# tayloraswift/swift-png

Measured on NVIDIA H100. Metric: MPixels/s decode (inflate+unfilter), higher is better.
Workload: dtype u8

## Files before the change

swift-png_b200/csrc/common.cuh:

```cuda
#pragma once

#ifdef PNGB200_EMU
#include "simt.h"
#else
#include <cuda_runtime.h>
#define PNGB200_DYN_SMEM(name) extern __shared__ __align__(16) unsigned char name[]
#endif
#include <stdint.h>

#include "../../include/pngb200.h"

namespace pngb200 {

struct StreamJob {
    const uint8_t* src;
    uint64_t       src_len;
    uint8_t*       dst;
    uint64_t       dst_cap;
    uint64_t       start_bit;
    uint64_t       start_out;
    int32_t        format;
    int32_t        phase;
    uint64_t       stop_bit;
    uint32_t       symbolic;
    uint32_t       may_switch;
    uint8_t*       scratch;
    uint64_t       scratch_cap;
};

struct StreamResult {
    int32_t  status;
    uint32_t err_a, err_b;
    uint32_t checksum;
    uint32_t blocks;
    uint32_t declared;
    uint64_t produced;
    uint64_t consumed_bits;
    uint64_t resume_bit;
    uint64_t resume_out;
    uint32_t trailer_seen;
    uint32_t phase;
    uint32_t stat_waves, stat_sync_rounds, stat_resolve_rounds, stat_fallback;
    uint64_t stat_tokens, stat_matches, stat_deferred;
    uint32_t ck_done;
    uint32_t pad_;
    uint64_t stat_cycles[12];
};

struct SwitchRecord {
    uint64_t out;
    uint64_t bytes;
};

struct ImageJob {
    const uint8_t*      filtered;
    uint8_t*            pixels;
    const StreamResult* inflated;
    uint64_t            filtered_len;
    uint32_t            width, height;
    uint32_t            pitch;
    uint8_t             volume, depth, interlaced, bpp;
};

__device__ __forceinline__ uint64_t usable_bytes(const StreamResult* r, uint64_t fallback)
{
    if (r == nullptr) return fallback;
    return r->status < 0 ? 0 : r->produced;
}

__device__ __forceinline__ unsigned lane_id() { return threadIdx.x & 31u; }

__device__ __forceinline__ uint32_t ld_volatile_u32(const uint32_t* p)
{
#ifdef PNGB200_EMU
    return *(const volatile uint32_t*)p;
#else
    uint32_t v;
    asm volatile("ld.volatile.global.u32 %0, [%1];" : "=r"(v) : "l"(p) : "memory");
    return v;
#endif
}
__device__ __forceinline__ void st_volatile_u32(uint32_t* p, uint32_t v)
{
#ifdef PNGB200_EMU
    *(volatile uint32_t*)p = v;
#else
    asm volatile("st.volatile.global.u32 [%0], %1;" ::"l"(p), "r"(v) : "memory");
#endif
}

}
```

swift-png_b200/csrc/huffman.cuh:

```cuda
#pragma once

#include "common.cuh"

namespace pngb200 {

enum : uint32_t { K_LIT = 0, K_BASE = 1, K_EOB = 2, K_PTR = 3, K_INVALID = 4 };
enum : uint32_t { E_COPY = 1u << 9, E_SPECIAL = 1u << 10, E_PTR = 1u << 11, E_INVALID = 2u << 11 };
__device__ __forceinline__ uint32_t mk_entry(uint32_t kind, uint32_t len, uint32_t extra, uint32_t value)
{
    uint32_t e = len | (len + extra) << 4 | value << 16;
    if (kind == K_BASE) e |= E_COPY;
    else if (kind == K_EOB) e |= E_SPECIAL;
    else if (kind == K_PTR) e |= E_SPECIAL | E_PTR;
    else if (kind == K_INVALID) e |= E_SPECIAL | E_INVALID;
    return e;
}
__device__ __forceinline__ uint32_t e_len(uint32_t e) { return e & 15u; }
__device__ __forceinline__ uint32_t e_skip(uint32_t e) { return (e >> 4) & 31u; }
__device__ __forceinline__ uint32_t e_extra(uint32_t e) { return e_skip(e) - e_len(e); }
__device__ __forceinline__ uint32_t e_kind(uint32_t e)
{
    return (e & E_SPECIAL) ? (((e >> 11) & 3u) == 0 ? K_EOB : ((e >> 11) & 3u) == 1 ? K_PTR : K_INVALID)
                           : ((e >> 9) & 1u);
}
__device__ __forceinline__ uint32_t e_value(uint32_t e) { return e >> 16; }

constexpr int LIT_ROOT  = 10;
constexpr int DIST_ROOT = 8;
constexpr int META_ROOT = 7;
constexpr int LIT_CAP   = (1 << LIT_ROOT) + 512;
constexpr int DIST_CAP  = (1 << DIST_ROOT) + 512;
constexpr int META_CAP  = 1 << META_ROOT;

__constant__ uint16_t c_len_base[29]  = {3, 4, 5, 6, 7, 8, 9, 10, 11, 13, 15, 17, 19, 23, 27,
                                         31, 35, 43, 51, 59, 67, 83, 99, 115, 131, 163, 195, 227, 258};
__constant__ uint8_t  c_len_extra[29] = {0, 0, 0, 0, 0, 0, 0, 0, 1, 1, 1, 1, 2, 2, 2,
                                         2, 3, 3, 3, 3, 4, 4, 4, 4, 5, 5, 5, 5, 0};
__constant__ uint16_t c_dist_base[30] = {1, 2, 3, 4, 5, 7, 9, 13, 17, 25, 33, 49, 65, 97, 129, 193,
                                         257, 385, 513, 769, 1025, 1537, 2049, 3073, 4097, 6145,
                                         8193, 12289, 16385, 24577};
__constant__ uint8_t  c_dist_extra[30] = {0, 0, 0, 0, 1, 1, 2, 2, 3, 3, 4, 4, 5, 5, 6, 6,
                                          7, 7, 8, 8, 9, 9, 10, 10, 11, 11, 12, 12, 13, 13};
__constant__ uint8_t  c_clen_order[19] = {16, 17, 18, 0, 8, 7, 9, 6, 10, 5, 11, 4, 12, 3, 13, 2, 14, 1, 15};

enum : int { ALPHA_LITLEN = 0, ALPHA_DIST = 1, ALPHA_META = 2 };

struct HuffScratch {
    uint32_t count[16];
    uint32_t first[16];
    uint32_t offs[16];
    uint32_t running[16];
    uint16_t sorted[320];
    uint32_t sub_alloc;
    int32_t  status;
    int32_t  stub;
};

__device__ __forceinline__ uint32_t symbol_entry(int alphabet, uint32_t sym, uint32_t len)
{
    if (alphabet == ALPHA_LITLEN) {
        if (sym < 256) return mk_entry(K_LIT, len, 0, sym);
        if (sym == 256) return mk_entry(K_EOB, len, 0, 0);
        if (sym < 286) return mk_entry(K_BASE, len, c_len_extra[sym - 257], c_len_base[sym - 257]);
        return mk_entry(K_INVALID, len, 0, sym);
    } else if (alphabet == ALPHA_DIST) {
        if (sym < 30) return mk_entry(K_BASE, len, c_dist_extra[sym], c_dist_base[sym]);
        return mk_entry(K_INVALID, len, 0, sym);
    }
    return mk_entry(K_LIT, len, 0, sym);
}

template <int ROOT, int CAP>
__device__ void build_table(uint32_t* table, const uint8_t* lens, int nsym, int alphabet,
                            HuffScratch* S, int tid, int nt)
{
    auto sync = [&]() {
        if (nt == 32) __syncwarp();
        else __syncthreads();
    };
    if (tid < 16) { S->count[tid] = 0; S->running[tid] = 0; }
    if (tid == 0) { S->sub_alloc = 1u << ROOT; S->status = 0; S->stub = -2; }
    sync();
    for (int s = tid; s < nsym; s += nt) atomicAdd(&S->count[lens[s]], 1u);
    sync();
    if (tid == 0) {
        int nonzero = nsym - (int)S->count[0];
        bool stub = false;
        if (alphabet == ALPHA_DIST) {
            if (nonzero == 0) { S->stub = -1; stub = true; }
            else if (nonzero == 1 && S->count[1] == 1) { S->stub = 0; stub = true; }
        }
        long interior = 1;
        uint32_t code = 0, off = 0;
        S->count[0] = 0;
        for (int l = 1; l <= 15; ++l) {
            code = (code + S->count[l - 1]) << 1;
            S->first[l] = code;
            S->offs[l] = off;
            off += S->count[l];
            interior = 2 * interior - (long)S->count[l];
        }
        if (!stub && interior != 0)
            S->status = alphabet == ALPHA_META ? PNGB200_ERR_CODELENGTH_HUFFMAN_TABLE
                                               : PNGB200_ERR_HUFFMAN_TABLE;
    }
    sync();
    if (S->status != 0) return;
    if (tid < 32) {
        for (int base = 0; base < nsym; base += 32) {
            int      s = base + tid;
            uint32_t l = s < nsym ? lens[s] : 0;
            unsigned peers = __match_any_sync(0xffffffffu, l);
            if (l) {
                uint32_t rank = __popc(peers & ((1u << tid) - 1u));
                uint32_t r0   = S->running[l];
                S->sorted[S->offs[l] + r0 + rank] = (uint16_t)s;
                __syncwarp(peers);
                if (rank == 0) S->running[l] = r0 + __popc(peers);
            }
            __syncwarp();
        }
    }
    sync();
    for (int i = tid; i < (1 << ROOT); i += nt) {
        uint32_t v = __brev((uint32_t)i) >> (32 - ROOT);
        uint32_t e = 0;
        bool     found = false;
#pragma unroll
        for (int l = 1; l <= ROOT; ++l) {
            uint32_t d = (v >> (ROOT - l)) - S->first[l];
            if (!found && d < S->count[l]) {
                e = symbol_entry(alphabet, S->sorted[S->offs[l] + d], (uint32_t)l);
                found = true;
            }
        }
        if (!found) {
            int maxl = 0;
            for (int l = ROOT + 1; l <= 15; ++l) {
                uint32_t lo = v << (l - ROOT), hi = (v + 1) << (l - ROOT);
                uint32_t a = S->first[l], b = a + S->count[l];
                if (S->count[l] && lo < b && a < hi) maxl = l;
            }
            if (maxl == 0) {
                e = mk_entry(K_INVALID, 0, 0, 0);
            } else {
                int      k    = maxl - ROOT;
                uint32_t slot = atomicAdd(&S->sub_alloc, 1u << k);
                if (slot + (1u << k) > (uint32_t)CAP) {
                    S->status = PNGB200_ERR_INTERNAL;
                    e = mk_entry(K_INVALID, 0, 0, 0);
                } else {
                    e = mk_entry(K_PTR, ROOT, (uint32_t)k, slot);
                    const uint32_t inv = mk_entry(K_INVALID, 0, 0, 0);
                    for (uint32_t j = 0; j < (1u << k); ++j) table[slot + j] = inv;
                }
            }
        }
        table[i] = e;
    }
    sync();
// ... 30 lines not shown
```

swift-png_b200/csrc/inflate_cells.cuh:

```cuda
#pragma once

#include "inflate_stream.cuh"

namespace pngb200 {

constexpr int      CL_CTAS_PER_SM = 3;
constexpr uint32_t CL_SLOTS       = 16000;
constexpr uint32_t CL_CAP         = CL_SLOTS - 16;
constexpr uint32_t CL_INWAVE      = 0xc000u;
constexpr uint32_t CL_WINDOW_BIAS = 0x8100u;
constexpr uint32_t CL_MIN_SUBS    = 32;
constexpr uint32_t CL_TCAP        = 64;
constexpr uint32_t CL_WCAP        = 64;
constexpr uint64_t CL_SCRATCH     = (uint64_t)WV_THREADS * (CL_TCAP + CL_WCAP) * sizeof(uint32_t);

struct ClShared {
    SerialShared ser;
    uint32_t     words[WV_SMEM_WORDS];
    uint32_t     mask[8 * WV_THREADS];
    uint32_t     pf_tail[16];
    uint32_t     exit_[WV_THREADS];
    uint32_t     wpos_[WV_THREADS];
    uint32_t     wn_[WV_THREADS];
    uint64_t     cross_[WV_THREADS];
// ... 17 lines not shown
static_assert(sizeof(ClShared) <= (228 * 1024 - CL_CTAS_PER_SM * 1024) / CL_CTAS_PER_SM, "CTAs per SM");
static_assert(CL_SLOTS <= 16384 && CL_SLOTS % 16 == 0, "14-bit cell index");

#ifdef PNGB200_EMU
inline void     sts16(saddr_t a, uint32_t v) { *(volatile uint16_t*)a = (uint16_t)v; }
inline uint32_t lds16(saddr_t a) { return *(volatile uint16_t*)a; }
inline void     sts32(saddr_t a, uint32_t v) { *(volatile uint32_t*)a = v; }
inline void     reds_or(saddr_t a, uint32_t v) { *(volatile uint32_t*)a |= v; }
#else
__device__ __forceinline__ void sts16(uint32_t a, uint32_t v)
{
    asm volatile("st.shared.u16 [%0], %1;" ::"r"(a), "h"((uint16_t)v) : "memory");
}
__device__ __forceinline__ uint32_t lds16(uint32_t a)
{
    uint16_t v;
    asm volatile("ld.shared.u16 %0, [%1];" : "=h"(v) : "r"(a) : "memory");
    return v;
}
__device__ __forceinline__ void sts32(uint32_t a, uint32_t v)
{
    asm volatile("st.shared.u32 [%0], %1;" ::"r"(a), "r"(v) : "memory");
}
__device__ __forceinline__ void reds_or(uint32_t a, uint32_t v)
{
    asm volatile("red.shared.or.b32 [%0], %1;" ::"r"(a), "r"(v) : "memory");
}
#endif
typedef saddr_t cellp_t;

__device__ __forceinline__ uint32_t cl_decode(FastBits& b, saddr_t lit, saddr_t dst, uint32_t& tok, uint32_t& nbytes, uint32_t& cp)
{
    const uint32_t bits = b.peek();
    uint32_t e = lds32(lit + ((bits & ((1u << LIT_ROOT) - 1u)) << 2));
    if (e & E_SPECIAL) {
        if ((e & (E_PTR | E_INVALID)) == E_PTR) e = lds32(lit + (((e >> 16) + bfe32(bits, LIT_ROOT, e_skip(e) - LIT_ROOT)) << 2));
        if (e & E_SPECIAL) {
            if (e & E_INVALID) return PF_BAD;
            b.skip(e_len(e));
            return PF_EOB;
        }
    }
    const uint32_t len = e & 15u, skipn = (e >> 4) & 31u;
    const uint32_t run = (e >> 16) + bfe32(bits, len, skipn - len);
    b.skip(skipn);
    cp = (e >> 9) & 1u;
    const uint32_t dbits = b.peek();
    uint32_t d = lds32(dst + ((dbits & ((1u << DIST_ROOT) - 1u)) << 2));
    if (d & E_SPECIAL) {
        if ((d & (E_PTR | E_INVALID)) == E_PTR) d = lds32(dst + (((d >> 16) + bfe32(dbits, DIST_ROOT, e_skip(d) - DIST_ROOT)) << 2));
        if (cp && (d & E_SPECIAL)) return PF_BAD;
    }
    const uint32_t dlen = d & 15u, dskip = (d >> 4) & 31u;
    const uint32_t dist = (d >> 16) + bfe32(dbits, dlen, dskip - dlen);
    b.skip(cp ? dskip : 0u);
    tok = run << 16 | (cp ? dist : 0u);
    nbytes = cp ? run : 1u;
    return 0;
}
__device__ __forceinline__ uint32_t tok_bytes(uint32_t v) { return (v & 0xffffu) ? v >> 16 : 1u; }

__device__ __forceinline__ void cells_copy(cellp_t ch, uint32_t j, uint32_t run, uint32_t dist, uint32_t jbeg)
{
    const int32_t src = (int32_t)j - (int32_t)dist;
    const saddr_t to = ch + 2 * j;
    if (src >= (int32_t)jbeg || src + (int32_t)run <= (int32_t)jbeg) {
        const uint32_t code = src >= (int32_t)jbeg ? CL_INWAVE + (uint32_t)src
                                                   : (uint32_t)((int32_t)CL_WINDOW_BIAS + src - (int32_t)jbeg);
        sts16(to, code);
        sts16(to + 2, code + 1);
        sts16(to + 4, code + 2);
        if (run > 3) sts16(to + 6, code + 3);
        for (uint32_t k = 4; k < run; ++k) sts16(to + 2 * k, code + k);
        return;
    }
    const uint32_t nwin = (uint32_t)((int32_t)jbeg - src);
    uint32_t code = (uint32_t)((int32_t)CL_WINDOW_BIAS + src - (int32_t)jbeg);
    uint32_t k = 0;
    for (; k < nwin; ++k) sts16(to + 2 * k, code + k);
    code = CL_INWAVE + (uint32_t)src;
    for (; k < run; ++k) sts16(to + 2 * k, code + k);
}

constexpr uint32_t CL_HDR_POS = 4480;

template <class Shared>
__device__ int cl_header_preamble(Shared& sh, uint64_t hbase_bit, uint64_t pos, uint64_t total_bits, int lane, WvHeader& out,
                                  uint32_t& rel_out)
{
    const uint32_t* const W = sh.words;
    auto get = [&](uint32_t rel, uint32_t n) -> uint32_t {
        const uint32_t w = rel >> 5;
        const uint32_t v = __funnelshift_r(W[w], W[w + 1], rel & 31u);
        return n >= 32 ? v : v & ((1u << n) - 1u);
    };
    uint32_t rel = (uint32_t)(pos - hbase_bit);
    if (pos + 3 > total_bits) return 0;
    const uint32_t h3 = get(rel, 3);
    rel += 3;
    out.status = PNGB200_OK;
    out.final = (int32_t)(h3 & 1u);
    out.type = (int32_t)(h3 >> 1);
    out.stored = 0;
    out.nlit = out.ndist = 0;
    if (out.type == 3) return 0;
    if (out.type == 0) {
        const uint64_t boundary = (pos + 3 + 7) & ~(uint64_t)7;
        if (boundary + 32 > total_bits) return 0;
        const uint32_t v = get((uint32_t)(boundary - hbase_bit), 32);
        const uint32_t l = v & 0xffffu, m = v >> 16;
        if (l != (~m & 0xffffu)) return 0;
        out.stored = l;
        out.pos = boundary + 32;
        return 1;
    }
    uint8_t* const lens = sh.ser.lens;
    if (out.type == 1) {
        for (int k = lane; k < 320; k += 32) lens[k] = k < 144 ? 8 : k < 256 ? 9 : k < 280 ? 7 : k < 288 ? 8 : 5;
        out.nlit = 288;
        out.ndist = 32;
        out.pos = pos + 3;
        __syncwarp();
        return 1;
    }
    if (pos + 17 > total_bits) return 0;
    const uint32_t v = get(rel, 14);
    rel += 14;
    const int nlit = 257 + (int)(v & 31u), ndist = 1 + (int)((v >> 5) & 31u), nclen = 4 + (int)(v >> 10);
    if (nlit > 286) return 0;
    if (lane < 19) lens[lane] = 0;
    __syncwarp();
    if (lane < nclen) lens[c_clen_order[lane]] = (uint8_t)get(rel + 3u * (uint32_t)lane, 3);
    rel += 3u * (uint32_t)nclen;
    __syncwarp();
    build_table<META_ROOT, META_CAP>(sh.ser.meta, lens, 19, ALPHA_META, &sh.ser.scratch, lane, 32);
    if (sh.ser.scratch.status) return 0;
    __syncwarp();
    if (rel + CL_HDR_POS + 64 > 32u * WV_HDR_WORDS) return 0;
    out.nlit = nlit;
    out.ndist = ndist;
    rel_out = rel;
    return 2;
}

__global__ void __launch_bounds__(WV_THREADS, CL_CTAS_PER_SM) inflate_cells_kernel(WvParams P)
{
    PNGB200_DYN_SMEM(cl_smem);
    ClShared& sh = *reinterpret_cast<ClShared*>(cl_smem);
    const uint32_t t    = threadIdx.x;
    const unsigned lane = lane_id(), warp = t >> 5;
    if (t == 0) mbar_init(&sh.pf_bar, 1);
    static_assert(offsetof(ClShared, pf_tail) == offsetof(ClShared, mask) + sizeof(uint32_t) * 8 * WV_THREADS &&
                  sizeof(uint32_t) * WV_PF_WORDS <= sizeof(uint32_t) * (8 * WV_THREADS + 16), "prefetch area = mask ++ pf_tail");
    static_assert(offsetof(ClShared, mask) % 16 == 0 && offsetof(ClShared, cells) % 32 == 0, "alignment");
    WavePrefetch pf{0, false, 0};
    const saddr_t sbase = opaque(smem_addr(cl_smem));
    const saddr_t words_addr = sbase + offsetof(ClShared, words);
    const saddr_t lit = sbase + offsetof(ClShared, ser) + offsetof(SerialShared, lit);
    const saddr_t dstt = sbase + offsetof(ClShared, ser) + offsetof(SerialShared, dist);
    const saddr_t mk_t = sbase + offsetof(ClShared, mask) + 4 * t;
    const saddr_t mk_0 = sbase + offsetof(ClShared, mask);
    uint32_t* const mk = sh.mask;
    cellp_t const ch = sbase + offsetof(ClShared, cells);
    uint32_t* const tok_own  = reinterpret_cast<uint32_t*>(P.scratch + blockIdx.x * P.scratch_stride);
    uint32_t* const tok_walk = tok_own + WV_THREADS * CL_TCAP;
    uint32_t* const tok_mine = tok_own + t * CL_TCAP;

    for (;;) {
        const int j = next_stream(sh, P);
        if (j < 0) return;
        StreamRun S;
        S.open(P, j);
        const StreamJob& job = S.job;
        StreamResult* const r = S.r;
        BitReader& br = S.br;
        uint64_t&  out = S.out;
        uint32_t waves = 0, sweep_rounds = 0, cuts = 0;
        uint64_t n_tokens = 0, n_matches = 0, walk_tokens = 0;
        uint8_t* const dst = job.dst;
        const bool     sym = job.symbolic != 0;
        uint16_t* const dst16 = reinterpret_cast<uint16_t*>(job.dst);
        uint32_t nsub = WV_THREADS;
        const bool adler_on = job.start_out == 0 && !sym;
        AdlerRun   adler;
        adler.reset();
        while (S.st == PNGB200_OK && S.phase == 1) {
            __syncthreads();
            adler.fold(sh);
            {
                const uint64_t hbase = br.pos >> 5;
                stage_header_words(sh, br);
                if (warp == 0) {
                    WvHeader h;
                    uint32_t rel = 0;
                    const int mode = cl_header_preamble(sh, hbase << 5, br.pos, br.total_bits, (int)lane, h, rel);
                    if (mode == 0) h = general_block_header(sh, br, r);
                    if (lane == 0) {
                        sh.hdr = h;
                        sh.hdr_mode = (uint32_t)mode;
                        sh.hdr_rel = rel;
                    }
                }
                __syncthreads();
                if (sh.hdr_mode == 2) {
                    const uint32_t rel = sh.hdr_rel;
                    const int      total_lens = sh.hdr.nlit + sh.hdr.ndist;
                    const saddr_t  tab = ch, list = ch + 4 * CL_HDR_POS;
                    const uint32_t* const W = sh.words;
                    for (uint32_t q = t; q < CL_HDR_POS; q += WV_THREADS) {
                        const uint32_t at = rel + q;
                        const uint32_t bits = __funnelshift_r(W[at >> 5], W[(at >> 5) + 1], at & 31u);
                        const uint32_t e = sh.ser.meta[bits & (META_CAP - 1)];
                        uint32_t word = 0;
                        if (!(e & E_SPECIAL)) {
                            const uint32_t len = e & 15u, sym = e >> 16, x = bits >> len;
                            word = sym < 16   ? (len | 1u << 8 | sym << 16)
                                 : sym == 16 ? ((len + 2u) | (3u + (x & 3u)) << 8 | 0xffu << 16)
                                 : sym == 17 ? ((len + 3u) | (3u + (x & 7u)) << 8)
                                             : ((len + 7u) | (11u + (x & 127u)) << 8);
                        }
                        sts32(tab + 4 * q, word);
                    }
                    __syncthreads();
                    if (t == 0) {
                        uint32_t p = 0, have = 0, prev = 0, count = 0, ok = 1;
                        while (have < (uint32_t)total_lens) {
// ... 498 lines not shown
```

swift-png_b200/csrc/inflate_serial.cuh:

```cuda
#pragma once

#include "huffman.cuh"

namespace pngb200 {

struct SerialShared {
    uint32_t    lit[LIT_CAP];
    uint32_t    dist[DIST_CAP];
    uint32_t    meta[META_CAP];
    uint8_t     lens[320 + 140];
    HuffScratch scratch;
};

struct BitReader {
    const uint32_t* words;
    uint64_t        lead_bits;
    uint64_t        total_bits;
    uint64_t        wi;
    uint64_t        buf;
    int             cnt;
    uint64_t        pos;

    __device__ void init(const uint8_t* src, uint64_t len, uint64_t start_bit)
    {
// ... 122 lines not shown
        uint32_t v = br.take(32);
        uint32_t l = v & 0xffff, m = v >> 16;
        if (l != (~m & 0xffffu)) return fail(r, PNGB200_ERR_BLOCK_COUNT_PARITY, l, m);
        br.refill();
        *stored_len = l;
        return PNGB200_OK;
    }
    if (*type == 3) return fail(r, PNGB200_ERR_BLOCK_TYPE, 3);
    int nlit, ndist;
    __syncwarp();
    if (*type == 1) {
        nlit = 288;
        ndist = 32;
        for (int s = lane; s < 320; s += 32)
            sh->lens[s] = s < 144 ? 8 : s < 256 ? 9 : s < 280 ? 7 : s < 288 ? 8 : 5;
    } else {
        if (!br.have(14)) return PNGB200_NEED_MORE_INPUT;
        br.refill();
        uint32_t v = br.take(14);
        nlit  = 257 + (int)(v & 31);
        ndist = 1 + (int)((v >> 5) & 31);
        int nclen = 4 + (int)(v >> 10);
        if (!br.have(3 * (uint64_t)nclen)) return PNGB200_NEED_MORE_INPUT;
        if (nlit > 286) return fail(r, PNGB200_ERR_RUNLITERAL_SYMBOL_COUNT, (uint32_t)nlit);
        if (lane < 19) sh->lens[lane] = 0;
        __syncwarp();
        for (int i = 0; i < nclen; ++i) {
            br.refill();
            uint32_t l = br.take(3);
            if (lane == 0) sh->lens[c_clen_order[i]] = (uint8_t)l;
        }
        __syncwarp();
        build_table<META_ROOT, META_CAP>(sh->meta, sh->lens, 19, ALPHA_META, &sh->scratch, lane, 32);
        if (sh->scratch.status) return fail(r, sh->scratch.status);
        int total = nlit + ndist, have = 0;
        uint32_t prev = 0;
        __syncwarp();
        while (have < total) {
            if (!br.have(1)) return PNGB200_NEED_MORE_INPUT;
            br.refill();
            uint32_t e = sh->meta[br.peek() & (META_CAP - 1)];
            uint32_t len = e_len(e), sym = e_value(e);
            if (!br.have(len)) return PNGB200_NEED_MORE_INPUT;
            if (sym < 16) {
                br.consume((int)len);
                if (lane == 0) sh->lens[have] = (uint8_t)sym;
                prev = sym;
                ++have;
                continue;
            }
            uint32_t element, extra, base;
            if (sym == 16) {
                if (have == 0) return fail(r, PNGB200_ERR_CODELENGTH_SEQUENCE);
                element = prev; extra = 2; base = 3;
            } else if (sym == 17) {
                element = 0; extra = 3; base = 3;
            } else {
                element = 0; extra = 7; base = 11;
            }
            if (!br.have(len + extra)) return PNGB200_NEED_MORE_INPUT;
            br.consume((int)len);
            uint32_t reps = base + br.take((int)extra);
            for (uint32_t k = lane; k < reps; k += 32) sh->lens[have + k] = (uint8_t)element;
            prev = element;
            have += (int)reps;
        }
        if (have != total) return fail(r, PNGB200_ERR_CODELENGTH_SEQUENCE);
    }
    __syncwarp();
    *nlit_out  = nlit;
    *ndist_out = ndist;
    return PNGB200_OK;
}

template <typename Shared>
__device__ int build_block_tables(Shared* sh, StreamResult* r, int nlit, int ndist, int tid, int nt)
{
    build_table<LIT_ROOT, LIT_CAP>(sh->lit, sh->lens, nlit, ALPHA_LITLEN, &sh->scratch, tid, nt);
    if (sh->scratch.status) return fail(r, sh->scratch.status);
    if (nt == 32) __syncwarp();
    else __syncthreads();
    build_table<DIST_ROOT, DIST_CAP>(sh->dist, sh->lens + nlit, ndist, ALPHA_DIST, &sh->scratch, tid, nt);
    if (sh->scratch.status) return fail(r, sh->scratch.status);
    return PNGB200_OK;
}

__device__ int read_trailer(BitReader& br, int format, StreamResult* r)
{
    if (format == PNGB200_FORMAT_IOS) {
        if (lane_id() == 0) r->trailer_seen = 1;
        return PNGB200_OK;
    }
    uint64_t boundary = (br.pos + 7) & ~(uint64_t)7;
    if (boundary + 32 > br.total_bits) return PNGB200_NEED_MORE_INPUT;
    br.seek(boundary);
    uint32_t v = br.take(32);
    uint32_t declared = format == PNGB200_FORMAT_GZIP ? v : __byte_perm(v, 0, 0x0123);
    if (lane_id() == 0) {
        r->declared     = declared;
        r->trailer_seen = 1;
    }
    if (format == PNGB200_FORMAT_GZIP) {
        if (!br.have(32)) return PNGB200_NEED_MORE_INPUT;
        br.refill();
        br.consume(32);
    }
    return PNGB200_OK;
}

__device__ void serial_inflate(SerialShared& sh, const StreamJob& job, StreamResult* r, uint64_t start_bit,
                               uint64_t start_out, uint32_t phase, uint32_t blocks)
{
    const unsigned lane = lane_id();
    BitReader      br;
    br.init(job.src, job.src_len, start_bit);
    uint64_t out = start_out;
    int      st  = PNGB200_OK;
    uint64_t resume_bit = start_bit, resume_out = start_out;

    if (phase == 0) {
        st = read_stream_header(br, job.format, r);
        if (st == PNGB200_OK) {
            resume_bit = br.at();
            phase = 1;
        }
    }
    uint8_t* dst = job.dst;
    if (st == PNGB200_OK && phase == 2) st = read_trailer(br, job.format, r);
    while (st == PNGB200_OK && phase == 1) {
        int      type, final;
        uint32_t stored = 0;
        int nlit = 0, ndist = 0;
        st = parse_block_header(br, &sh, r, (int)lane, &type, &final, &stored, &nlit, &ndist);
        if (st == PNGB200_OK && type != 0) st = build_block_tables(&sh, r, nlit, ndist, (int)lane, 32);
        if (st != PNGB200_OK) break;
        if (type == 0) {
            if (!br.have(8 * (uint64_t)stored)) { st = PNGB200_NEED_MORE_INPUT; break; }
            if (out + stored > job.dst_cap) { st = fail(r, PNGB200_ERR_OUTPUT_CAPACITY); break; }
            const uint8_t* s = job.src + (br.at() >> 3);
            for (uint32_t k = lane; k < stored; k += 32) dst[out + k] = s[k];
            out += stored;
            br.seek(br.pos + 8 * (uint64_t)stored);
            __syncwarp();
        } else {
            for (;;) {
                br.refill();
                uint32_t e   = lookup<LIT_ROOT>(sh.lit, br.peek());
                uint32_t len = e_len(e), kind = e_kind(e);
                if (kind == K_LIT) {
                    if (!br.have(len)) { st = PNGB200_NEED_MORE_INPUT; break; }
                    if (out >= job.dst_cap) { st = fail(r, PNGB200_ERR_OUTPUT_CAPACITY); break; }
                    br.consume((int)len);
                    if (lane == 0) dst[out] = (uint8_t)e_value(e);
                    ++out;
                } else if (kind == K_BASE) {
                    uint64_t start = br.pos;
                    br.consume((int)len);
                    uint32_t run = e_value(e) + br.take((int)e_extra(e));
                    br.refill();
                    uint32_t d = lookup<DIST_ROOT>(sh.dist, br.peek());
                    if (e_kind(d) != K_BASE) {
                        if (start + len + e_extra(e) + e_len(d) > br.total_bits) st = PNGB200_NEED_MORE_INPUT;
                        else st = fail(r, PNGB200_ERR_INVALID_SYMBOL, e_value(d), 1);
                        break;
                    }
                    br.consume((int)e_len(d));
// ... 53 lines not shown
```

swift-png_b200/csrc/inflate_stream.cuh:

```cuda
#pragma once

#include "inflate_serial.cuh"

namespace pngb200 {

constexpr int      WV_THREADS      = 256;
constexpr int      WV_WARPS        = WV_THREADS / 32;
constexpr uint32_t WV_SUB_BITS     = 256;
constexpr uint32_t WV_BITS         = WV_THREADS * WV_SUB_BITS;
constexpr uint32_t WV_WORDS        = WV_BITS / 32 + 8;
constexpr uint32_t WV_SMEM_WORDS   = WV_WORDS + WV_WORDS / 8 + 1;
constexpr uint32_t WV_WINDOW       = 32768;
constexpr uint32_t WV_HDR_WORDS    = 192;
constexpr uint32_t ADLER_MOD32     = 65521;
constexpr uint32_t WV_WALK_K       = 8;

#if defined(PNGB200_EMU) && defined(WV_PROFILE)
struct WvProfile { uint64_t thread_iters[8], warp_iters[8]; };
inline WvProfile& wv_profile() { static WvProfile p; return p; }
inline void wv_count(int phase, uint32_t iters)
{
    uint32_t m = iters;
    for (int o = 16; o; o >>= 1) m = max(m, __shfl_xor_sync(0xffffffffu, m, o));
    wv_profile().thread_iters[phase] += iters;
// ... 508 lines not shown
        } else if (t == 0) {
            if (r->status == 0) r->status = st;
            r->produced      = out;
            r->consumed_bits = br.at();
            r->blocks        = blocks;
            r->resume_bit    = resume_bit;
            r->resume_out    = resume_out;
            r->phase         = phase;
            if (adler_on) adler.check_trailer(r, job.format);
        }
        if (t == 0) r->stat_fallback = fallback ? 1u : 0u;
    }
};

template <class Shared>
__device__ __forceinline__ void report_wave_stats(Shared& sh, StreamResult* r, uint32_t waves, uint64_t matches, uint64_t tokens,
                                                  uint64_t deferred, uint64_t walk_tokens, uint32_t rounds)
{
    const unsigned warp = threadIdx.x >> 5;
    for (int o = 16; o; o >>= 1) {
        tokens += __shfl_down_sync(0xffffffffu, tokens, o);
        deferred += __shfl_down_sync(0xffffffffu, deferred, o);
        walk_tokens += __shfl_down_sync(0xffffffffu, walk_tokens, o);
        rounds = max(rounds, __shfl_down_sync(0xffffffffu, rounds, o));
    }
    if (lane_id() == 0) {
        sh.warp_sums[warp] = tokens;
        sh.adler_a[warp] = (uint32_t)min(deferred, (uint64_t)0xffffffffu);
        sh.adler_b[warp] = (uint32_t)min(walk_tokens, (uint64_t)0xffffffffu);
        sh.exc[warp] = rounds;
    }
    __syncthreads();
    if (threadIdx.x == 0) {
        uint64_t tk = 0, df = 0, wt = 0;
        uint32_t rr = 0;
        for (int w = 0; w < WV_WARPS; ++w) {
            tk += sh.warp_sums[w];
            df += sh.adler_a[w];
            wt += sh.adler_b[w];
            rr = max(rr, sh.exc[w]);
        }
        r->stat_waves          = waves;
        r->stat_sync_rounds    = (uint32_t)min(wt, (uint64_t)0xffffffffu);
        r->stat_resolve_rounds = rr;
        r->stat_tokens         = tk;
        r->stat_matches        = matches;
        r->stat_deferred       = df;
        for (int k = 0; k < 12; ++k) r->stat_cycles[k] = sh.cyc[k];
    }
}

template <class Shared>
__device__ WvHeader general_block_header(Shared& sh, const BitReader& br, StreamResult* r)
{
    int      type = 0, final = 0, nlit = 0, ndist = 0;
    uint32_t stored = 0;
    StagedReader sr;
    sr.init(sh.words, (br.pos >> 5) << 5, br.total_bits, br.pos);
    const int st = parse_block_header(sr, &sh.ser, r, (int)lane_id(), &type, &final, &stored, &nlit, &ndist);
    return WvHeader{st, type, final, nlit, ndist, stored, sr.pos};
}

template <class Shared>
__device__ __forceinline__ void stage_header_words(Shared& sh, const BitReader& br)
{
    const uint64_t hbase = br.pos >> 5;
    for (uint32_t k = threadIdx.x; k < WV_HDR_WORDS; k += WV_THREADS) sh.words[k] = br.load_word(hbase + k);
    __syncthreads();
}

template <class Shared>
__device__ __forceinline__ WvHeader read_block_header(Shared& sh, const BitReader& br, StreamResult* r)
{
    stage_header_words(sh, br);
    if (threadIdx.x < 32) {
        WvHeader h;
        if (!wv_fast_header(sh, (br.pos >> 5) << 5, br.pos, br.total_bits, (int)lane_id(), h)) h = general_block_header(sh, br, r);
        if (lane_id() == 0) sh.hdr = h;
    }
    __syncthreads();
    return sh.hdr;
}

template <class Shared>
__device__ __forceinline__ uint64_t cta_scan_packed(Shared& sh, uint64_t mine)
{
    const unsigned lane = lane_id(), warp = threadIdx.x >> 5;
    uint64_t incl = mine;
    for (int o = 1; o < 32; o <<= 1) {
        uint64_t v = __shfl_up_sync(0xffffffffu, incl, o);
        if ((int)lane >= o) incl += v;
    }
    if (lane == 31) sh.warp_sums[warp] = incl;
    __syncthreads();
    if (warp == 0) {
        uint64_t ws = lane < WV_WARPS ? sh.warp_sums[lane] : 0, wi = ws;
        for (int o = 1; o < 32; o <<= 1) {
            uint64_t v = __shfl_up_sync(0xffffffffu, wi, o);
            if ((int)lane >= o) wi += v;
        }
        if (lane < WV_WARPS) sh.warp_sums[lane] = wi - ws;
        if (lane == WV_WARPS - 1) sh.warp_sums[WV_WARPS] = wi;
    }
    __syncthreads();
    return sh.warp_sums[warp] + incl - mine;
}


struct WavePrefetch {
    uint32_t parity;
    bool     pending;
    uint64_t first;

    template <class Shared>
    __device__ __forceinline__ void drain(Shared& sh)
    {
        if (pending) {
            while (!mbar_try_wait(&sh.pf_bar, parity)) {}
            parity ^= 1;
            pending = false;
        }
    }
    template <class Shared>
    __device__ __forceinline__ void start(Shared& sh, const BitReader& br, uint64_t nbase)
    {
        const uint64_t f = nbase - ((((uintptr_t)br.words >> 2) + nbase) & 3);
        if (f >= 1 && (f + WV_PF_WORDS + 1) * 32 <= br.total_bits) {
            if (threadIdx.x == 0) {
                fence_proxy_async();
                mbar_expect_tx(&sh.pf_bar, sizeof(uint32_t) * WV_PF_WORDS);
                bulk_g2s(sh.mask, br.words + f, sizeof(uint32_t) * WV_PF_WORDS, &sh.pf_bar);
            }
            pending = true;
            first = f;
        }
    }
    template <class Shared>
    __device__ __forceinline__ void stage(Shared& sh, const BitReader& br, uint64_t wbase)
    {
        const bool had = pending;
        drain(sh);
        if (had && wbase >= first && wbase - first < 4) {
            const uint32_t* lin = sh.mask + (uint32_t)(wbase - first);
            for (uint32_t k = threadIdx.x; k < WV_WORDS; k += WV_THREADS) sh.words[k + (k >> 3)] = lin[k];
        } else {
            for (uint32_t k = threadIdx.x; k < WV_WORDS; k += WV_THREADS) sh.words[k + (k >> 3)] = br.load_word(wbase + k);
        }
    }
};

template <class Shared>
__device__ __forceinline__ void follow_chain(Shared& sh)
{
    uint32_t E[WV_WARPS];
#pragma unroll
    for (int w = 0; w < WV_WARPS; ++w) E[w] = sh.exc[w];
    uint32_t cur = 0, x = 0;
    bool     done = false;
#pragma unroll
    for (int w = 0; w < WV_WARPS; ++w) {
        uint32_t v = 0;
        while (!done && cur < 32u * (w + 1)) {
            const uint32_t lo = cur - 32u * w;
            const uint32_t m = E[w] & (~0u << lo);
            if (m == 0) {
                v |= ~0u << lo;
// ... 30 lines not shown
```

swift-png_b200/csrc/inflate_wave.cuh:

```cuda
#pragma once

#include "inflate_stream.cuh"

namespace pngb200 {

constexpr int      WV_CTAS_PER_SM  = 2;
constexpr uint32_t WV_RING         = 65536;
constexpr uint32_t WV_OUT_BYTES    = WV_RING - WV_WINDOW;
constexpr uint32_t WV_BITMAP_WORDS = WV_OUT_BYTES / 32;
constexpr uint32_t WV_LIST_CAP     = WV_BITS / 2 + 64;
constexpr unsigned WV_POLL_NS      = 20;

struct WvShared {
    SerialShared ser;
    uint32_t     words[WV_SMEM_WORDS];
    uint32_t     mask[8 * WV_THREADS];
    uint32_t     ck[8 * WV_THREADS];
    uint32_t     exit_[WV_THREADS];
    uint32_t     wpos_[WV_THREADS];
    uint32_t     wn_[WV_THREADS];
    uint64_t     cross_[WV_THREADS];
    uint16_t     wc_[WV_THREADS];
    uint16_t     next_[WV_THREADS];
    uint8_t      kind_[WV_THREADS];
// ... 101 lines not shown
    uint32_t  first;
    uint32_t  clean;
    uint32_t  c_next;
    bool      bad_ref;
};

template <bool IN_HBM>
__device__ __forceinline__ void emit_token(EmitState& S, uint32_t run, uint32_t dist, uint32_t is_copy)
{
    const uint32_t o = S.o;
    if (!is_copy) {
        if (IN_HBM) S.hbm[o] = (uint8_t)run;
        else S.ring[(S.rbase + o) & 0xffffu] = (uint8_t)run;
        S.o = o + 1;
        return;
    }
    if (dist > S.reach + o) {
        S.bad_ref = true;
        return;
    }
    const int32_t src = (int32_t)o - (int32_t)dist;
    bool final = src + (int32_t)run <= 0 || src >= (int32_t)S.clean;
    if (!final && src >= (int32_t)S.first)
        final = bits_all_clear(S.U, (uint32_t)src, min(run, dist));
    if (final) {
        if (IN_HBM) hbm_copy(S.hbm, o, run, dist);
        else ring_copy(S.ring, S.rbase + o, S.rbase + o - dist, run, dist);
    } else {
        bits_set(S.U, o, run);
        S.list[S.c_next++] = CopyItem{o, run | (dist - 1) << 16};
        S.clean = o + run;
    }
    S.o = o + run;
}

__device__ __forceinline__ void emit_token_sym(EmitState& S, uint32_t run, uint32_t dist, uint32_t is_copy)
{
    uint16_t* const h = reinterpret_cast<uint16_t*>(S.hbm);
    uint32_t o = S.o;
    if (!is_copy) {
        h[o] = (uint16_t)run;
        S.o = o + 1;
        return;
    }
    const uint32_t have = S.reach + o;
    if (dist > have) {
        const uint32_t pre = min(dist - have, run);
        const uint32_t idx = WV_WINDOW - (dist - have);
        for (uint32_t k = 0; k < pre; ++k) h[o + k] = (uint16_t)(0x8000u | (idx + k));
        o += pre;
        run -= pre;
        if (run == 0) { S.o = o; return; }
    }
    const int32_t src = (int32_t)o - (int32_t)dist;
    bool final = src + (int32_t)run <= 0 || src >= (int32_t)S.clean;
    if (!final && src >= (int32_t)S.first) final = bits_all_clear(S.U, (uint32_t)src, min(run, dist));
    if (final) {
        hbm_copy(h, o, run, dist);
    } else {
        bits_set(S.U, o, run);
        S.list[S.c_next++] = CopyItem{o, run | (dist - 1) << 16};
        S.clean = o + run;
    }
    S.o = o + run;
}

__global__ void __launch_bounds__(WV_THREADS, WV_CTAS_PER_SM) inflate_wave_kernel(WvParams P)
{
    PNGB200_DYN_SMEM(wv_smem);
    WvShared& sh = *reinterpret_cast<WvShared*>(wv_smem);
    const uint32_t t    = threadIdx.x;
    const unsigned lane = lane_id(), warp = t >> 5;
    CopyItem* const list    = reinterpret_cast<CopyItem*>(P.scratch + blockIdx.x * P.scratch_stride);
    uint32_t* const gbitmap = reinterpret_cast<uint32_t*>(P.scratch + blockIdx.x * P.scratch_stride +
                                                         sizeof(CopyItem) * WV_LIST_CAP);
    for (uint32_t k = t; k < WV_BITMAP_WORDS; k += WV_THREADS) sh.bitmap[k] = 0;
    if (t == 0) mbar_init(&sh.pf_bar, 1);
    static_assert(offsetof(WvShared, ck) == offsetof(WvShared, mask) + sizeof(uint32_t) * 8 * WV_THREADS, "prefetch area = mask ++ ck");
    static_assert(sizeof(uint32_t) * WV_PF_WORDS <= 2 * sizeof(uint32_t) * 8 * WV_THREADS && offsetof(WvShared, mask) % 16 == 0, "prefetch area");
    WavePrefetch pf{0, false, 0};
    const saddr_t words_addr = smem_addr(sh.words);
    const saddr_t lit = smem_addr(sh.ser.lit), dstt = smem_addr(sh.ser.dist);
    uint32_t* const mk = sh.mask;

    for (;;) {
        const int j = next_stream(sh, P);
        if (j < 0) return;
        StreamRun S;
        S.open(P, j);
        const StreamJob& job = S.job;
        StreamResult* const r = S.r;
        BitReader& br = S.br;
        uint64_t&  out = S.out;
        uint32_t waves = 0, resolve_rounds = 0;
        uint64_t n_tokens = 0, n_matches = 0, n_deferred = 0, walk_tokens = 0;
        uint8_t* dst     = job.dst;
        uint64_t dst_cap = job.dst_cap;
        bool     sym     = job.symbolic != 0;
        uint32_t esz     = sym ? 2u : 1u;
        uint32_t mis     = (uint32_t)((uintptr_t)dst & 15);
        const bool may_switch = sym && job.may_switch;
        uint64_t   mark_end = 0, sw_out = ~0ull, sw_bytes = 0;
        bool over_cap = false;
        bool ring_stale = job.start_out != 0;
        const bool adler_on = job.start_out == 0 && !sym;
        AdlerRun   adler;
        adler.reset();
        auto try_switch = [&]() {
            if (!may_switch || !sym || out < mark_end + WV_WINDOW) return;
            const uint64_t area = (2 * out + 15) & ~(uint64_t)15;
            const uint64_t room = 2 * job.dst_cap;
            if (area + WV_WINDOW > room) return;
            const uint16_t* const s16 = reinterpret_cast<const uint16_t*>(job.dst);
            uint8_t* const        nd  = job.dst + area + WV_WINDOW - out;
            for (uint64_t x = out - WV_WINDOW + t; x < out; x += WV_THREADS) nd[x] = (uint8_t)s16[x];
            __syncthreads();
            sym        = false;
            esz        = 1;
            dst        = nd;
            dst_cap    = room - area - WV_WINDOW + out;
            mis        = (uint32_t)((uintptr_t)nd & 15);
            ring_stale = true;
            sw_out     = out;
            sw_bytes   = area + WV_WINDOW;
        };

        while (S.st == PNGB200_OK && S.phase == 1) {
            __syncthreads();
            adler.fold(sh);
            const WvHeader hdr = read_block_header(sh, br, r);
            S.st = hdr.status;
            if (S.st != PNGB200_OK) break;
            const int      type = hdr.type, final = hdr.final;
            const uint32_t stored = hdr.stored;
            br.seek(hdr.pos);
            if (type != 0) {
                S.st = build_block_tables(&sh.ser, r, hdr.nlit, hdr.ndist, (int)t, WV_THREADS);
                if (S.st != PNGB200_OK) break;
            }
            phase_tick(sh, 0);
            if (type == 0) {
                if (!S.copy_stored(sh, dst, dst_cap, sym, stored, adler, adler_on)) break;
                if (stored) ring_stale = true;
                try_switch();
                phase_tick(sh, 9);
            } else {
                bool block_done = false;
                while (!block_done) {
                    ++waves;
                    const uint64_t wstart = br.pos;
                    const uint64_t wbase  = (wstart >> 5) & ~(uint64_t)7;
                    __syncthreads();
                    pf.stage(sh, br, wbase);
                    if (t == 0) sh.wcount[0] = 0;
                    __syncthreads();
                    adler.fold(sh);
                    phase_tick(sh, 1);
                    const uint32_t rel0  = (uint32_t)(wstart - (wbase << 5));
                    const uint32_t base  = t * WV_SUB_BITS;
                    const uint32_t limit = base + WV_SUB_BITS;

                    uint32_t nout = 0, ncopy = 0, flags = 0, exit_bit;
                    {
#pragma unroll
                        for (int k = 0; k < 8; ++k) mk[k * WV_THREADS + t] = 0;
                        sh.ck[t] = 0;
                        FastBits b;
                        b.init(words_addr, t == 0 ? rel0 : base);
                        uint32_t mi = 0, mw = 0, n = 0;
                        while (b.pos < limit) {
                            const uint32_t rr = b.pos - base, wi = rr >> 5;
                            if (wi != mi) {
                                mk[mi * WV_THREADS + t] = mw;
                                mw = 0;
                                mi = wi;
                                sh.ck[wi * WV_THREADS + t] = nout | ncopy << 16;
                            }
                            mw |= 1u << (rr & 31);
                            uint32_t run = 0, dist = 0, cp = 0;
                            const uint32_t s = wv_decode<false>(b, lit, dstt, run, dist, cp);
                            if (s) { flags = s; break; }
                            nout += cp ? run : 1u;
                            ncopy += cp;
                            ++n;
                        }
                        mk[mi * WV_THREADS + t] = mw;
                        exit_bit = b.pos;
                        WV_COUNT(0, n);
                    }
                    sh.exit_[t] = exit_bit;
                    sh.cross_[t] = 0;
                    __syncthreads();
                    phase_tick(sh, 2);

                    {
                        uint32_t u = t, pos = exit_bit, wn = 0, wc = 0;
                        bool     active = flags == 0;
                        if (!active) {
                            sh.kind_[t] = (uint8_t)(flags == PF_EOB ? WK_OWN_EOB : WK_OWN_BAD);
                            sh.wpos_[t] = exit_bit;
                            sh.wn_[t] = 0;
                            sh.wc_[t] = 0;
                        }
                        for (uint32_t round = 0;; ++round) {
                            const uint32_t K = WV_WALK_K << min(round, 6u);
                            bool     still = false;
                            uint32_t iters = 0;
                            if (active) {
                                FastBits b;
                                b.init(words_addr, pos);
                                uint32_t kind = WK_RUNNING;
                                const uint32_t first_sub = sh.exit_[u] >> 8;
                                bool     crossed = sh.cross_[u] != 0;
                                for (; iters < K; ++iters) {
                                    const uint32_t p = b.pos;
                                    if (p >= WV_BITS) { kind = WK_END; break; }
                                    const uint32_t s = p >> 8, rr = p & 255u;
                                    if (!crossed && s > first_sub) {
                                        sh.cross_[u] = 1ull << 63 | (uint64_t)p << 40 | (uint64_t)(wc & 0xffu) << 24 | (wn & 0xffffffu);
                                        crossed = true;
                                    }
                                    if ((mk[(rr >> 5) * WV_THREADS + s] >> (rr & 31)) & 1u) { kind = WK_SYNC; break; }
                                    uint32_t run = 0, dist = 0, cp = 0;
                                    const uint32_t e = wv_decode<false>(b, lit, dstt, run, dist, cp);
                                    if (e) { kind = e == PF_EOB ? WK_EOB : WK_BAD; break; }
                                    wn += cp ? run : 1u;
                                    wc += cp;
                                }
                                sh.wpos_[u] = b.pos;
                                sh.wn_[u]   = wn;
                                sh.wc_[u]   = (uint16_t)wc;
                                sh.kind_[u] = (uint8_t)kind;
                                still = kind == WK_RUNNING;
                                walk_tokens += iters;
                            }
                            WV_COUNT(1, iters);
// ... 293 lines not shown
```

Before: 11280.

## Parallelize dynamic block header decode and split lit/dist table builds across named barriers

Replaces the single-warp block header read in the wave kernel with a CTA-wide version. It reuses already-staged input words when they are available, decodes code-length symbols speculatively at every bit position in parallel, and then stitches them with a paired-step serial walk followed by a parallel fill of the lengths. The literal/length and distance Huffman tables are now built at the same time by disjoint thread groups that synchronise on separate named barriers (bar.sync ids 1 and 2). This is meant to cut the serial per-block header latency, at the cost of more shared-memory reuse of the mask area, extra CTA barriers, and a fallback path when the speculation window is exceeded.

Result: no change. 11330, median of 6 (+0.5%).

```diff
diff --git a/swift-png_b200/csrc/common.cuh b/swift-png_b200/csrc/common.cuh
--- a/swift-png_b200/csrc/common.cuh
+++ b/swift-png_b200/csrc/common.cuh
@@ -2,6 +2,9 @@
 
 #ifdef PNGB200_EMU
 #include "simt.h"
+
+#include <map>
+#include <utility>
 #else
 #include <cuda_runtime.h>
 #define PNGB200_DYN_SMEM(name) extern __shared__ __align__(16) unsigned char name[]
@@ -70,6 +73,34 @@
 
 __device__ __forceinline__ unsigned lane_id() { return threadIdx.x & 31u; }
 
+#ifdef PNGB200_EMU
+inline void bar_sync(unsigned id, unsigned n)
+{
+    struct Named { unsigned at = 0; uint64_t gen = 0; };
+    static std::map<std::pair<const void*, unsigned>, Named> bars;
+    simt::Fiber* const f = simt::self();
+    if (id == 0 || id > 15 || n == 0 || n % 32 || n > f->cta->nthreads) {
+        fprintf(stderr, "bar.sync %u, %u: invalid\n", id, n);
+        abort();
+    }
+    Named& b = bars[{f->cta, id}];
+    const uint64_t gen = b.gen;
+    f->wait = "bar.sync";
+    f->wait_arg = id;
+    if (++b.at >= n) {
+        b.at = 0;
+        ++b.gen;
+        return;
+    }
+    while (b.gen == gen) simt::yield();
+}
+#else
+__device__ __forceinline__ void bar_sync(unsigned id, unsigned n)
+{
+    asm volatile("bar.sync %0, %1;" ::"r"(id), "r"(n) : "memory");
+}
+#endif
+
 __device__ __forceinline__ uint32_t ld_volatile_u32(const uint32_t* p)
 {
 #ifdef PNGB200_EMU
diff --git a/swift-png_b200/csrc/huffman.cuh b/swift-png_b200/csrc/huffman.cuh
--- a/swift-png_b200/csrc/huffman.cuh
+++ b/swift-png_b200/csrc/huffman.cuh
@@ -72,10 +72,11 @@
 
 template <int ROOT, int CAP>
 __device__ void build_table(uint32_t* table, const uint8_t* lens, int nsym, int alphabet,
-                            HuffScratch* S, int tid, int nt)
+                            HuffScratch* S, int tid, int nt, int bar = 0)
 {
     auto sync = [&]() {
         if (nt == 32) __syncwarp();
+        else if (bar) bar_sync((unsigned)bar, (unsigned)nt);
         else __syncthreads();
     };
     if (tid < 16) { S->count[tid] = 0; S->running[tid] = 0; }
diff --git a/swift-png_b200/csrc/inflate_cells.cuh b/swift-png_b200/csrc/inflate_cells.cuh
--- a/swift-png_b200/csrc/inflate_cells.cuh
+++ b/swift-png_b200/csrc/inflate_cells.cuh
@@ -123,66 +123,6 @@
     for (; k < run; ++k) sts16(to + 2 * k, code + k);
 }
 
-constexpr uint32_t CL_HDR_POS = 4480;
-
-template <class Shared>
-__device__ int cl_header_preamble(Shared& sh, uint64_t hbase_bit, uint64_t pos, uint64_t total_bits, int lane, WvHeader& out,
-                                  uint32_t& rel_out)
-{
-    const uint32_t* const W = sh.words;
-    auto get = [&](uint32_t rel, uint32_t n) -> uint32_t {
-        const uint32_t w = rel >> 5;
-        const uint32_t v = __funnelshift_r(W[w], W[w + 1], rel & 31u);
-        return n >= 32 ? v : v & ((1u << n) - 1u);
-    };
-    uint32_t rel = (uint32_t)(pos - hbase_bit);
-    if (pos + 3 > total_bits) return 0;
-    const uint32_t h3 = get(rel, 3);
-    rel += 3;
-    out.status = PNGB200_OK;
-    out.final = (int32_t)(h3 & 1u);
-    out.type = (int32_t)(h3 >> 1);
-    out.stored = 0;
-    out.nlit = out.ndist = 0;
-    if (out.type == 3) return 0;
-    if (out.type == 0) {
-        const uint64_t boundary = (pos + 3 + 7) & ~(uint64_t)7;
-        if (boundary + 32 > total_bits) return 0;
-        const uint32_t v = get((uint32_t)(boundary - hbase_bit), 32);
-        const uint32_t l = v & 0xffffu, m = v >> 16;
-        if (l != (~m & 0xffffu)) return 0;
-        out.stored = l;
-        out.pos = boundary + 32;
-        return 1;
-    }
-    uint8_t* const lens = sh.ser.lens;
-    if (out.type == 1) {
-        for (int k = lane; k < 320; k += 32) lens[k] = k < 144 ? 8 : k < 256 ? 9 : k < 280 ? 7 : k < 288 ? 8 : 5;
-        out.nlit = 288;
-        out.ndist = 32;
-        out.pos = pos + 3;
-        __syncwarp();
-        return 1;
-    }
-    if (pos + 17 > total_bits) return 0;
-    const uint32_t v = get(rel, 14);
-    rel += 14;
-    const int nlit = 257 + (int)(v & 31u), ndist = 1 + (int)((v >> 5) & 31u), nclen = 4 + (int)(v >> 10);
-    if (nlit > 286) return 0;
-    if (lane < 19) lens[lane] = 0;
-    __syncwarp();
-    if (lane < nclen) lens[c_clen_order[lane]] = (uint8_t)get(rel + 3u * (uint32_t)lane, 3);
-    rel += 3u * (uint32_t)nclen;
-    __syncwarp();
-    build_table<META_ROOT, META_CAP>(sh.ser.meta, lens, 19, ALPHA_META, &sh.ser.scratch, lane, 32);
-    if (sh.ser.scratch.status) return 0;
-    __syncwarp();
-    if (rel + CL_HDR_POS + 64 > 32u * WV_HDR_WORDS) return 0;
-    out.nlit = nlit;
-    out.ndist = ndist;
-    rel_out = rel;
-    return 2;
-}
 
 __global__ void __launch_bounds__(WV_THREADS, CL_CTAS_PER_SM) inflate_cells_kernel(WvParams P)
 {
diff --git a/swift-png_b200/csrc/inflate_serial.cuh b/swift-png_b200/csrc/inflate_serial.cuh
--- a/swift-png_b200/csrc/inflate_serial.cuh
+++ b/swift-png_b200/csrc/inflate_serial.cuh
@@ -228,6 +228,18 @@
     else __syncthreads();
     build_table<DIST_ROOT, DIST_CAP>(sh->dist, sh->lens + nlit, ndist, ALPHA_DIST, &sh->scratch, tid, nt);
     if (sh->scratch.status) return fail(r, sh->scratch.status);
+    return PNGB200_OK;
+}
+
+template <class Shared>
+__device__ int build_block_tables_split(Shared* sh, HuffScratch* dscratch, StreamResult* r, int nlit, int ndist, int tid, int nt)
+{
+    const int nl = nt - 64;
+    if (tid < nl) build_table<LIT_ROOT, LIT_CAP>(sh->lit, sh->lens, nlit, ALPHA_LITLEN, &sh->scratch, tid, nl, 1);
+    else build_table<DIST_ROOT, DIST_CAP>(sh->dist, sh->lens + nlit, ndist, ALPHA_DIST, dscratch, tid - nl, 64, 2);
+    __syncthreads();
+    if (sh->scratch.status) return fail(r, sh->scratch.status);
+    if (dscratch->status) return fail(r, dscratch->status);
     return PNGB200_OK;
 }
 
diff --git a/swift-png_b200/csrc/inflate_stream.cuh b/swift-png_b200/csrc/inflate_stream.cuh
--- a/swift-png_b200/csrc/inflate_stream.cuh
+++ b/swift-png_b200/csrc/inflate_stream.cuh
@@ -614,6 +614,194 @@
     return sh.hdr;
 }
 
+constexpr uint32_t CL_HDR_POS = 2240;
+
+struct HdrArea {
+    uint16_t    tab[CL_HDR_POS];
+    uint32_t    pair[CL_HDR_POS];
+    uint32_t    list[320];
+    HuffScratch dscratch;
+    uint32_t    mode, rel, ok, count;
+};
+__device__ __forceinline__ uint32_t hdr_lengths(uint32_t e) { return e >> 8 ? e >> 8 : 1u; }
+__device__ __forceinline__ bool     hdr_is_repeat(uint32_t e) { return (e >> 8) && ((e >> 4) & 15u); }
+__device__ __forceinline__ uint32_t hdr_value(uint32_t e, uint32_t prev)
+{
+    return hdr_is_repeat(e) ? prev : (e >> 8) ? 0u : (e >> 4) & 15u;
+}
+
+template <class Shared>
+__device__ int cl_header_preamble(Shared& sh, uint64_t hbase_bit, uint64_t pos, uint64_t total_bits, int lane, WvHeader& out,
+                                  uint32_t& rel_out)
+{
+    const uint32_t* const W = sh.words;
+    auto get = [&](uint32_t rel, uint32_t n) -> uint32_t {
+        const uint32_t w = rel >> 5;
+        const uint32_t v = __funnelshift_r(W[w], W[w + 1], rel & 31u);
+        return n >= 32 ? v : v & ((1u << n) - 1u);
+    };
+    uint32_t rel = (uint32_t)(pos - hbase_bit);
+    if (pos + 3 > total_bits) return 0;
+    const uint32_t h3 = get(rel, 3);
+    rel += 3;
+    out.status = PNGB200_OK;
+    out.final = (int32_t)(h3 & 1u);
+    out.type = (int32_t)(h3 >> 1);
+    out.stored = 0;
+    out.nlit = out.ndist = 0;
+    if (out.type == 3) return 0;
+    if (out.type == 0) {
+        const uint64_t boundary = (pos + 3 + 7) & ~(uint64_t)7;
+        if (boundary + 32 > total_bits) return 0;
+        const uint32_t v = get((uint32_t)(boundary - hbase_bit), 32);
+        const uint32_t l = v & 0xffffu, m = v >> 16;
+        if (l != (~m & 0xffffu)) return 0;
+        out.stored = l;
+        out.pos = boundary + 32;
+        return 1;
+    }
+    uint8_t* const lens = sh.ser.lens;
+    if (out.type == 1) {
+        for (int k = lane; k < 320; k += 32) lens[k] = k < 144 ? 8 : k < 256 ? 9 : k < 280 ? 7 : k < 288 ? 8 : 5;
+        out.nlit = 288;
+        out.ndist = 32;
+        out.pos = pos + 3;
+        __syncwarp();
+        return 1;
+    }
+    if (pos + 17 > total_bits) return 0;
+    const uint32_t v = get(rel, 14);
+    rel += 14;
+    const int nlit = 257 + (int)(v & 31u), ndist = 1 + (int)((v >> 5) & 31u), nclen = 4 + (int)(v >> 10);
+    if (nlit > 286) return 0;
+    if (lane < 19) lens[lane] = 0;
+    __syncwarp();
+    if (lane < nclen) lens[c_clen_order[lane]] = (uint8_t)get(rel + 3u * (uint32_t)lane, 3);
+    rel += 3u * (uint32_t)nclen;
+    __syncwarp();
+    build_table<META_ROOT, META_CAP>(sh.ser.meta, lens, 19, ALPHA_META, &sh.ser.scratch, lane, 32);
+    if (sh.ser.scratch.status) return 0;
+    __syncwarp();
+    if (rel + CL_HDR_POS + 64 > 32u * WV_HDR_WORDS) return 0;
+    out.nlit = nlit;
+    out.ndist = ndist;
+    rel_out = rel;
+    return 2;
+}
+
+template <class Shared>
+__device__ void cta_code_lengths(Shared& sh, HdrArea& A, const BitReader& br, StreamResult* r, uint64_t hbase)
+{
+    const uint32_t t = threadIdx.x;
+    const uint32_t rel = A.rel;
+    const uint32_t total = (uint32_t)(sh.hdr.nlit + sh.hdr.ndist);
+    const uint32_t* const W = sh.words;
+    for (uint32_t q = t; q < CL_HDR_POS; q += WV_THREADS) {
+        const uint32_t at = rel + q;
+        const uint32_t bits = __funnelshift_r(W[at >> 5], W[(at >> 5) + 1], at & 31u);
+        const uint32_t e = sh.ser.meta[bits & (META_CAP - 1)];
+        uint32_t v = 0;
+        if (!(e & E_SPECIAL)) {
+            const uint32_t len = e & 15u, sym = e >> 16, x = bits >> len;
+            v = sym < 16   ? (len | sym << 4)
+              : sym == 16 ? ((len + 2u) | 1u << 4 | (3u + (x & 3u)) << 8)
+              : sym == 17 ? ((len + 3u) | (3u + (x & 7u)) << 8)
+                          : ((len + 7u) | (11u + (x & 127u)) << 8);
+        }
+        A.tab[q] = (uint16_t)v;
+    }
+    __syncthreads();
+    for (uint32_t q = t; q < CL_HDR_POS; q += WV_THREADS) {
+        const uint32_t e1 = A.tab[q], a1 = e1 & 15u;
+        uint32_t pr = 0;
+        if (a1 && q + a1 < CL_HDR_POS) {
+            const uint32_t e2 = A.tab[q + a1], a2 = e2 & 15u;
+            if (a2) {
+                const bool     def = !hdr_is_repeat(e1) || !hdr_is_repeat(e2);
+                const uint32_t val = !hdr_is_repeat(e2) ? hdr_value(e2, 0) : hdr_value(e1, 0);
+                pr = (a1 + a2) | (hdr_lengths(e1) + hdr_lengths(e2)) << 5 | (uint32_t)def << 14 | val << 15;
+            }
+        }
+        A.pair[q] = pr;
+    }
+    __syncthreads();
+    if (t == 0) {
+        uint32_t p = 0, have = 0, prev = 0, count = 0, ok = 1;
+        while (have < total) {
+            const uint32_t e2 = A.pair[p], e1 = A.tab[p];
+            const uint32_t n2 = (e2 >> 5) & 511u, n1 = hdr_lengths(e1);
+            if ((e1 & 15u) == 0 || (have == 0 && hdr_is_repeat(e1))) { ok = 0; break; }
+            const bool two = e2 != 0 && have + n2 <= total;
+            if (!two && have + n1 > total) { ok = 0; break; }
+            A.list[count++] = have | p << 9 | prev << 21 | (uint32_t)two << 25;
+            if (two) {
+                if ((e2 >> 14) & 1u) prev = (e2 >> 15) & 15u;
+                p += e2 & 31u;
+                have += n2;
+            } else {
+                prev = hdr_value(e1, prev);
+                p += e1 & 15u;
+                have += n1;
+            }
+            if (p >= CL_HDR_POS) { ok = 0; break; }
+        }
+        const uint64_t end = (hbase << 5) + rel + p;
+        if (end > br.total_bits) ok = 0;
+        A.ok = ok;
+        A.count = count;
+        sh.hdr.pos = end;
+    }
+    __syncthreads();
+    if (A.ok) {
+        uint8_t* const lens = sh.ser.lens;
+        for (uint32_t i = t; i < A.count; i += WV_THREADS) {
+            const uint32_t l = A.list[i];
+            const uint32_t at = l & 511u, p = (l >> 9) & 4095u;
+            const uint32_t e1 = A.tab[p], n1 = hdr_lengths(e1), v1 = hdr_value(e1, (l >> 21) & 15u);
+            for (uint32_t k = 0; k < n1; ++k) lens[at + k] = (uint8_t)v1;
+            if ((l >> 25) & 1u) {
+                const uint32_t e2 = A.tab[p + (e1 & 15u)], n2 = hdr_lengths(e2), v2 = hdr_value(e2, v1);
+                for (uint32_t k = 0; k < n2; ++k) lens[at + n1 + k] = (uint8_t)v2;
+            }
+        }
+    } else if (t < 32) {
+        const WvHeader h = general_block_header(sh, br, r);
+        if (lane_id() == 0) sh.hdr = h;
+    }
+    __syncthreads();
+}
+
+template <class Shared>
+__device__ WvHeader cta_block_header(Shared& sh, HdrArea& A, const BitReader& br, StreamResult* r, uint64_t staged)
+{
+    static_assert(WV_HDR_WORDS <= WV_THREADS, "one header word per thread");
+    const uint32_t t = threadIdx.x;
+    const uint64_t hbase = br.pos >> 5;
+    if (hbase >= staged && hbase - staged + WV_HDR_WORDS <= WV_WORDS) {
+        const uint32_t s = (uint32_t)(hbase - staged) + t;
+        const uint32_t v = t < WV_HDR_WORDS ? sh.words[s + (s >> 3)] : 0u;
+        __syncthreads();
+        if (t < WV_HDR_WORDS) sh.words[t] = v;
+        __syncthreads();
+    } else {
+        stage_header_words(sh, br);
+    }
+    if (t < 32) {
+        WvHeader h;
+        uint32_t rel = 0;
+        const int mode = cl_header_preamble(sh, hbase << 5, br.pos, br.total_bits, (int)lane_id(), h, rel);
+        if (mode == 0) h = general_block_header(sh, br, r);
+        if (lane_id() == 0) {
+            sh.hdr = h;
+            A.mode = (uint32_t)mode;
+            A.rel = rel;
+        }
+    }
+    __syncthreads();
+    if (A.mode == 2) cta_code_lengths(sh, A, br, r, hbase);
+    return sh.hdr;
+}
+
 template <class Shared>
 __device__ __forceinline__ uint64_t cta_scan_packed(Shared& sh, uint64_t mine)
 {
diff --git a/swift-png_b200/csrc/inflate_wave.cuh b/swift-png_b200/csrc/inflate_wave.cuh
--- a/swift-png_b200/csrc/inflate_wave.cuh
+++ b/swift-png_b200/csrc/inflate_wave.cuh
@@ -207,6 +207,8 @@
     const saddr_t words_addr = smem_addr(sh.words);
     const saddr_t lit = smem_addr(sh.ser.lit), dstt = smem_addr(sh.ser.dist);
     uint32_t* const mk = sh.mask;
+    static_assert(sizeof(HdrArea) <= 2 * sizeof(uint32_t) * 8 * WV_THREADS, "header work area = mask ++ ck");
+    HdrArea& hA = *reinterpret_cast<HdrArea*>(sh.mask);
 
     for (;;) {
         const int j = next_stream(sh, P);
@@ -250,17 +252,20 @@
             sw_bytes   = area + WV_WINDOW;
         };
 
+        uint64_t staged = ~0ull;
         while (S.st == PNGB200_OK && S.phase == 1) {
             __syncthreads();
             adler.fold(sh);
-            const WvHeader hdr = read_block_header(sh, br, r);
+            pf.drain(sh);
+            const WvHeader hdr = cta_block_header(sh, hA, br, r, staged);
+            staged = ~0ull;
             S.st = hdr.status;
             if (S.st != PNGB200_OK) break;
             const int      type = hdr.type, final = hdr.final;
             const uint32_t stored = hdr.stored;
             br.seek(hdr.pos);
             if (type != 0) {
-                S.st = build_block_tables(&sh.ser, r, hdr.nlit, hdr.ndist, (int)t, WV_THREADS);
+                S.st = build_block_tables_split(&sh.ser, &hA.dscratch, r, hdr.nlit, hdr.ndist, (int)t, WV_THREADS);
                 if (S.st != PNGB200_OK) break;
             }
             phase_tick(sh, 0);
@@ -277,6 +282,7 @@
                     const uint64_t wbase  = (wstart >> 5) & ~(uint64_t)7;
                     __syncthreads();
                     pf.stage(sh, br, wbase);
+                    staged = wbase;
                     if (t == 0) sh.wcount[0] = 0;
                     __syncthreads();
                     adler.fold(sh);
```
